# emiliofidalgo/liodom

Measured on AMD Instinct MI355X. Metric: scans/sec (64×1800 cloud, prev_frames=20) at 1 GPU; pose RMSE vs CPU ref, higher is better.
Workload: dtype f64

## Files before the change

### liodom_amd/csrc/kernels_lm.h

```cpp
constexpr int kLmWaves = kLmThreads / 64;


__device__ int lm_compact_bits(const DevView& v, int s, int outer_it, int E, int* idx ) {
  const int lane = threadIdx.x & 63;
  const int Q = v.knn_queries;
  const int nb = (E + Q - 1) / Q;
  const int nwords = (nb + 3) >> 2;
  const unsigned int* mw = reinterpret_cast<const unsigned int*>(v.corr_mask + ((size_t)s * 2 + outer_it) * v.mask_stride);
  int run = 0;
  for (int w0 = 0; w0 < nwords; w0 += 64) {
    const int w = w0 + lane;
    unsigned int word = (w < nwords) ? mw[w] : 0u;
    const int pop = __popc(word);
    const int incl = wave_incl_scan_i32(pop);
    int o = run + incl - pop;
    while (word) {
      const int b = __ffs(word) - 1;
      word &= word - 1u;
      const int bit = w * 32 + b;
      idx[o++] = (bit >> 3) * Q + (bit & 7);
    }
    run += readlane_i32(incl, 63);
  }
  return run;
// ... 325 lines not shown
  __shared__ int sh_spec_at;
  if (threadIdx.x == 77) sh_spec_at = st.spec_eval[outer_it];
  __shared__ int sh_redo;
  if (threadIdx.x == 78) sh_redo = st.spec_redo[outer_it == 0 ? 1 : 0];
  extern __shared__ __attribute__((aligned(16))) int sh_idx[];
  const int tid = threadIdx.x;
  const bool prep = tid < kLmCtl;
  bool dead = false;
  if (chain && outer_it == 0) dead = !chain_wait_count(v.knn_done0 + s, done_target, &st.status);
  if (chain && outer_it == 0 && sh_redo) __builtin_amdgcn_fence(__ATOMIC_ACQUIRE, "agent");
  int E_in;
  if (chain && outer_it == 0) {
    typedef __attribute__((address_space(1))) unsigned int gu32;
    E_in = (int)__hip_atomic_load((gu32*)(v.edge_cnt + eb * 32 + s), __ATOMIC_RELAXED, __HIP_MEMORY_SCOPE_AGENT);
  } else {
    E_in = st.n_edges_buf[eb];
  }
  if (outer_it == 0 && tid == 0 && g == 0) {
    st.info.n_edges = E_in;
    st.info.map_points = st.n_search;
    for (int k = 0; k < 2; k++) {
      st.info.lm[k].iterations = 0; st.info.lm[k].accepted = 0; st.info.lm[k].termination = LM_TERM_NO_RESIDUALS;
      st.info.lm[k].pad = 0; st.info.lm[k].initial_cost = 0.0; st.info.lm[k].final_cost = 0.0;
    }
  }
  if (!st.initialized) {
    if (outer_it == 1 && g == 0) {
      if (seq) ov_wait_knn_done(v, s, seq, &st.status);
      if (tid == 0) st.append_raw = 1;
      __shared__ double sh_T0[12];
      if (tid < 12) sh_T0[tid] = st.odom[tid];
      __syncthreads();
      finalize_scan(v, s, st, sh_cnt, eb, true, 0, 0, sh_T0, 1, true, sh_prev, sh_fc);
      if (tid == 0) st.initialized = 1;
      if (v.cov_raw && tid == 64) {
        PoseCovRaw* r = v.cov_raw + s;
        r->scan_index = st.info.scan_index; r->n_res = 0; r->termination = st.info.lm[1].termination; r->has_solve = 0; r->cost = st.info.lm[1].final_cost;
      }
    }
    return;
  }
  bool clr_pending = outer_it == 1 && g == 0 && prep && !v.early_rebuild;
  auto clear_hash_slots = [&]() {
    hash_clear_used(v, s, st.n_used_tab[0], tid, kLmCtl);
    clr_pending = false;
  };
  const bool dbgb = (s == 0) && (g == 0) && (tid == kLmCtl) && (outer_it == 1);
  const bool dbge = (s == 0) && (g == 0) && (tid == 0) && (outer_it == 1);
  DBG_STAMP(v, dbgb, 2, 0);
  const int E = E_in;
  int nblocks = st.info.matches[outer_it];
  __shared__ int sh_nmatch;
  __shared__ double sh_scale[8];
  const unsigned int epoch0 = ((unsigned int)(st.scan_counter + 1) << 6) | ((unsigned int)outer_it << 5);
  unsigned int n_eval = 0;
  bool xch_local = false;
  LmCache cache;
  int c_lo = 0, c_hi = 0;
  int dbg_it = 0;
  auto evaluate = [&](const double* pose) {
    lm_eval(v, s, outer_it, eb, c_lo, c_hi, sh_idx, pose, &sh_wsum[0][0], cache);
    if (tid >= kLmCtl) {
      const int lane = tid - kLmCtl;
      if (G > 1) {
        const double x = lm_wave_total(&sh_wsum[0][0], c_hi - c_lo, lane >> 1);
        DBG_STAMP(v, dbgb && dbg_it < 4, 2, 12 + dbg_it);
        xch_local = lm_exchange(v, s, g, G, epoch0 | ++n_eval, x, sh_acc, &st.status, xch_local, lane);
      } else {
        if (lane < kAccN) sh_acc[lane] = lm_wave_total(&sh_wsum[0][0], c_hi - c_lo, lane);
        ++n_eval;
      }
      asm volatile("s_waitcnt lgkmcnt(0)" ::: "memory");
      __builtin_amdgcn_wave_barrier();
    }
  };
  auto my_share = [&](int C) {
    const int chunk = (C + G - 1) / G;
    c_lo = g * chunk < C ? g * chunk : C;
    c_hi = (g + 1) * chunk < C ? (g + 1) * chunk : C;
  };
  if (seq && outer_it == 1) { if (chain) dead = !chain_wait_count(v.knn_done0 + 32 + s, done_target, &st.status) || dead; else ov_wait_knn_done(v, s, seq, &st.status); }
  if (seq && outer_it == 1) { __syncthreads(); if (sh_redo) __builtin_amdgcn_fence(__ATOMIC_ACQUIRE, "agent"); }
  OV_STAMP(v, g == 0 && tid == 0 && outer_it == 1, 4);
  OV_STAMP(v, g == 0 && tid == 0 && outer_it == 0, 18);
  if (v.knn_partials) {
    const int Q = v.knn_queries;
    const int nb = (E + Q - 1) / Q;
    const double* part = v.knn_part + ((size_t)s * 2 + outer_it) * v.knn_blocks * 32;
    constexpr int kRC = kLmThreads / 32;
    const int i = tid & 31, r0 = tid >> 5;
    double x0 = 0.0, x1 = 0.0;
    if (i <= kAccN) {
      const int nb_cap = v.knn_blocks;
      for (int rb = r0; rb < (dead ? 0 : (rb == r0 ? nb_cap : nb)); rb += 16 * kRC) {
        double xs[16];
#pragma unroll
        for (int u = 0; u < 16; u++) { const int r = rb + kRC * u; xs[u] = (r < nb_cap) ? part[(size_t)r * 32 + i] : 0.0; }
#pragma unroll
        for (int u = 0; u < 16; u++) { const int r = rb + kRC * u; if (r >= nb) xs[u] = 0.0; }
#pragma unroll
        for (int u = 0; u < 16; u += 2) { x0 += xs[u]; x1 += xs[u + 1]; }
      }
    }
    sh_red[r0][i] = x0 + x1;
    __syncthreads();
    if (tid <= kAccN) {
      double x = 0.0;
#pragma unroll
      for (int r = 0; r < kRC; r++) x += sh_red[r][tid];
      if (tid < kAccN) sh_acc[tid] = x;
      else { sh_nmatch = (int)x; if (g == 0) st.info.matches[outer_it] = (int)x; }
    }
    __syncthreads();
    nblocks = sh_nmatch;
  } else {
    __syncthreads();
    if (prep) {
      const int C = lm_compact_bits(v, s, outer_it, E, sh_idx);
      if (tid == 0) sh_C = C;
    } else if (tid == kLmCtl) {
      iso_from_qt(sh_x0, sh_x0 + 4, sh_pose2[0]);
    }
    __syncthreads();
    my_share(sh_C);
    lm_cache_load(v, s, outer_it, eb, c_lo, c_hi, sh_idx, cache);
    evaluate(sh_pose2[0]);
  }
  DBG_STAMP(v, dbgb, 2, 2);
  int pi = 0, ci = -1, nmoved = 0;
  const unsigned int n_eval0 = n_eval;
  const bool spec_ok = v.speculate != 0 && v.speculate != 5 && v.speculate != 7 && g == 0 && seq != 0u && outer_it == 0;
  const bool spec_ok1 = v.speculate != 0 && v.speculate != 4 && v.speculate != 6 && g == 0 && chain != 0 && outer_it == 1 && v.early_rebuild && v.pred_xch != nullptr;
  const bool spec_forced = v.speculate == 2 || v.speculate == 6 || v.speculate == 7;
  bool spec_done = false;
  int spec_moves = -1;
  for (int step = 0;; step++) {
    if (step == 0 && tid > kLmCtl && tid <= kLmCtl + 6) {
      const int j = tid - kLmCtl - 1;
      sh_scale[j] = 1.0 / (1.0 + sqrt(sh_acc[7 + h_idx(j, j)]));
    }
    if (step == 0) __builtin_amdgcn_wave_barrier();
    if (tid == kLmCtl) {
      const int acc_before = step == 0 ? 0 : lm.accepted;
      const int f = step == 0 ? lm_begin(lm, sh_x0, sh_x0 + 4, sh_acc, nblocks, v.apply_on_ftol, sh_scale) : lm_update(lm, sh_acc);
      sh_flag = f;
      bool moved = step > 0 && lm.accepted != acc_before;
      if (step > 0 && !moved && f != LM_NEED_EVAL && lm.termination == LM_TERM_FUNC_TOL) {
        moved = true;
        for (int k = 0; k < 4; k++) moved = moved && lm.q[k] == lm.cand_q[k];
        for (int k = 0; k < 3; k++) moved = moved && lm.t[k] == lm.cand_t[k];
      }
      if (moved) { ci = pi; pi ^= 1; nmoved++; }
      if (f == LM_NEED_EVAL) iso_from_qt(lm.cand_q, lm.cand_t, sh_pose2[pi]);
      sh_pi = pi; sh_ci = ci; sh_nmoved = nmoved; sh_unapplied = (step > 0 && !moved) ? 1 : 0;
      if (step == 0) DBG_STAMP(v, dbgb, 2, 23);
    } else if (!prep) {
    } else if (step == 0 && v.knn_partials) {
      DBG_STAMP(v, dbge, 2, 24);
      const int C = dead ? 0 : lm_compact_bits(v, s, outer_it, E, sh_idx);
      if (tid == 0) sh_C = C;
      DBG_STAMP(v, dbge, 2, 25);
      my_share(C);
      lm_cache_load(v, s, outer_it, eb, c_lo, c_hi, sh_idx, cache);
    } else if (clr_pending) {
      clear_hash_slots();
    }
    __syncthreads();
    if (step == 0) { if (v.knn_partials && !prep) my_share(sh_C); DBG_STAMP(v, dbgb, 2, 3); }
    else { DBG_STAMP(v, dbgb && dbg_it < 5, 2, 5 + 2 * dbg_it); dbg_it++; }
    if (sh_flag != LM_NEED_EVAL) break;
    if ((spec_ok || spec_ok1) && !spec_done && sh_ci >= 0 &&
        (spec_forced || (!spec_forced && sh_spec_at == 0 && lm.model_cost_change <= v.spec_theta * 1e-6 * lm.cost))) {
      if (spec_ok) {
        ov_publish_pose(v, s, sh_pose2[sh_ci], &lm.q[0], seq, tid, 1);
        OV_STAMP(v, tid == 0, 19);
      } else if (tid >= kLmCtl) {
        const int l = tid - kLmCtl;
        if (l < 25) publish_final_pose(v, s, sh_pose2[sh_ci], 0, (unsigned int)sh_fc + 1u, l, 0);
        if (l == 0) predict_next(sh_pose2[sh_ci], sh_prev, v.rotation_mode, sh_pred_s);
        asm volatile("s_waitcnt lgkmcnt(0)" ::: "memory");
        __builtin_amdgcn_wave_barrier();
        pred_publish(v, s, sh_pred_s, (unsigned int)sh_fc + 1u, l, 64, 1);
        OV_STAMP(v, l == 0, 22);
      }
      if ((kInstrument && (v.debug & 64)) && tid == 0) atomicAdd(&v.dbg_clk[270], 1ull);
      spec_done = true;
      spec_moves = sh_nmoved;
    }
    const double* pose_c = sh_pose2[sh_pi];
    evaluate(pose_c);
    DBG_STAMP(v, dbgb && dbg_it < 5, 2, 4 + 2 * dbg_it);
  }
  if (clr_pending) clear_hash_slots();
  DBG_STAMP(v, dbgb, 2, 20);
  if ((kInstrument && (v.debug & 32)) && dbgb) v.dbg_clk[2 * 32 + 27] = (xch_local ? 100ull : 0ull) + 10ull * xcc_id() + (unsigned long long)n_eval;
  if (g != 0) return;
  __shared__ double sh_ov[20];
  __shared__ liodom_lm_trace_t sh_trace;
  {
    if (tid == kLmCtl) {
      sh_trace.iterations = lm.iter; sh_trace.accepted = lm.accepted; sh_trace.termination = lm.termination; sh_trace.pad = 0;
      sh_trace.initial_cost = lm.initial_cost; sh_trace.final_cost = lm.cost;
    }
    const int cif = sh_ci;
    if (cif >= 0) {
      if (tid < 12) sh_ov[tid] = sh_pose2[cif][tid];
      else if (tid >= 64 && tid < 71) sh_ov[12 + tid - 64] = (&lm.q[0])[tid - 64];
    } else if (tid == kLmCtl) {
      double q[4], t[3], T[12];
      for (int k = 0; k < 4; k++) q[k] = lm.q[k];
      for (int k = 0; k < 3; k++) t[k] = lm.t[k];
      iso_from_qt(q, t, T);
      for (int k = 0; k < 12; k++) sh_ov[k] = T[k];
      for (int k = 0; k < 4; k++) sh_ov[12 + k] = q[k];
      for (int k = 0; k < 3; k++) sh_ov[16 + k] = t[k];
    }
  }
  __syncthreads();
  if (outer_it == 0) {
    if (seq) { ov_publish_pose(v, s, sh_ov, sh_ov + 12, seq, tid, spec_done ? 2 : 3); OV_STAMP(v, tid == 0, 1); }
// ... 25 lines not shown
```

### liodom_amd/csrc/liodom_math.h

```cpp
#pragma once
#include <cfloat>
#include <cmath>
#include <cstdint>

#if defined(__HIPCC__)
#define LD_HD __host__ __device__ __forceinline__
#define LD_UNROLL _Pragma("unroll")
#define LD_FP_CONTRACT_FAST _Pragma("clang fp contract(fast)")
#else
#define LD_HD inline
#define LD_UNROLL
#define LD_FP_CONTRACT_FAST
#endif
#if defined(__HIP_DEVICE_COMPILE__)
#define LD_RSQRT(x) rsqrt(x)
#else
#define LD_RSQRT(x) (1.0 / sqrt(x))
#endif

namespace liodom_dev {

constexpr int kJacobiSweeps = 8;
constexpr int kLmMaxIterations = 4;
constexpr double kHuberA = 0.2;
// ... 238 lines not shown
  m[6] = -sj;     m[7] = cj * si;      m[8] = cj * ci;
}
LD_HD void tf_quat_from_matrix(const double* m, double* q) {
  const double trace = m[0] + m[4] + m[8];
  if (trace > 0.0) {
    double s = sqrt(trace + 1.0);
    q[3] = s * 0.5;
    s = 0.5 / s;
    q[0] = (m[7] - m[5]) * s;
    q[1] = (m[2] - m[6]) * s;
    q[2] = (m[3] - m[1]) * s;
  } else {
    const int i = m[0] < m[4] ? (m[4] < m[8] ? 2 : 1) : (m[0] < m[8] ? 2 : 0);
    const int j = (i + 1) % 3, k = (i + 2) % 3;
    double s = sqrt(m[i * 3 + i] - m[j * 3 + j] - m[k * 3 + k] + 1.0);
    q[i] = s * 0.5;
    s = 0.5 / s;
    q[3] = (m[k * 3 + j] - m[j * 3 + k]) * s;
    q[j] = (m[j * 3 + i] + m[i * 3 + j]) * s;
    q[k] = (m[k * 3 + i] + m[i * 3 + k]) * s;
  }
}
LD_HD void imu_override(const double* odom, const double* imu_q, const double* laser_to_base, int rotation_mode, double* out) {
  double m[9], imu_roll, imu_pitch, imu_yaw, bl_roll, bl_pitch, bl_yaw;
  tf_matrix_from_quat(imu_q, m);
  tf_get_rpy(m, &imu_roll, &imu_pitch, &imu_yaw);
  double odom_bl[12], q_bl[4], q_new[4], l2b_inv[12];
  iso_mul(odom, laser_to_base, odom_bl);
  quat_from_pose(odom_bl, rotation_mode, q_bl);
  tf_matrix_from_quat(q_bl, m);
  tf_get_rpy(m, &bl_roll, &bl_pitch, &bl_yaw);
  tf_set_rpy(imu_roll, imu_pitch, bl_yaw, m);
  tf_quat_from_matrix(m, q_new);
  const double t_bl[3] = {odom_bl[3], odom_bl[7], odom_bl[11]};
  iso_from_qt(q_new, t_bl, odom_bl);
  iso_inverse(laser_to_base, l2b_inv);
  iso_mul(odom_bl, l2b_inv, out);
}
LD_HD void odom_message(const double* prev_odom, const double* odom, const double* laser_to_base,
                        double delta_time, int rotation_mode, double* out) {
  double bl[12], pbl[12], pinv[12], d[12], qd[4], m[9], roll, pitch, yaw;
  iso_mul(odom, laser_to_base, bl);
  quat_from_pose(bl, rotation_mode, out);
  out[4] = bl[3]; out[5] = bl[7]; out[6] = bl[11];
  iso_mul(prev_odom, laser_to_base, pbl);
  iso_inverse(pbl, pinv);
  iso_mul(pinv, bl, d);
  out[7] = d[3] / delta_time; out[8] = d[7] / delta_time; out[9] = d[11] / delta_time;
  quat_from_pose(d, rotation_mode, qd);
  tf_matrix_from_quat(qd, m);
  tf_get_rpy(m, &roll, &pitch, &yaw);
  out[10] = roll / delta_time; out[11] = pitch / delta_time; out[12] = yaw / delta_time;
}
LD_HD void quat_plus(const double* x, const double* delta, double* out) {
  LD_FP_CONTRACT_FAST
  const double u2 = delta[0] * delta[0] + delta[1] * delta[1] + delta[2] * delta[2];
  if (u2 > 0.0) {
    double s, aw;
    if (u2 < 0.25) {
      const double u = u2;
      s = 1.0 + u * (-1.0 / 6.0 + u * (1.0 / 120.0 + u * (-1.0 / 5040.0 + u * (1.0 / 362880.0 + u * (-1.0 / 39916800.0 +
          u * (1.0 / 6227020800.0 + u * (-1.0 / 1307674368000.0 + u * (1.0 / 355687428096000.0))))))));
      aw = 1.0 + u * (-0.5 + u * (1.0 / 24.0 + u * (-1.0 / 720.0 + u * (1.0 / 40320.0 + u * (-1.0 / 3628800.0 +
           u * (1.0 / 479001600.0 + u * (-1.0 / 87178291200.0 + u * (1.0 / 20922789888000.0))))))));
    } else {
      const double nd = sqrt(u2);
      s = sin(nd) / nd;
      aw = cos(nd);
    }
    const double ax = s * delta[0], ay = s * delta[1], az = s * delta[2];
    const double bw = x[3], bx = x[0], by = x[1], bz = x[2];
    out[3] = aw * bw - ax * bx - ay * by - az * bz;
    out[0] = aw * bx + ax * bw + ay * bz - az * by;
    out[1] = aw * by + ay * bw + az * bx - ax * bz;
    out[2] = aw * bz + az * bw + ax * by - ay * bx;
  } else {
    out[0] = x[0]; out[1] = x[1]; out[2] = x[2]; out[3] = x[3];
  }
}

LD_HD float sqdist_f(float qx, float qy, float qz, float mx, float my, float mz) {
  const float dx = qx - mx, dy = qy - my, dz = qz - mz;
  float r = dx * dx;
  r = r + dy * dy;
  r = r + dz * dz;
  return r;
}

LD_HD void jacobi_rot(double& app, double& aqq, double& apq, double& arp, double& arq) {
  if (fabs(apq) <= 1e-20 * (fabs(app) + fabs(aqq))) return;
  const double theta = (aqq - app) / (2.0 * apq);
  const double at = fabs(theta);
  double t = 1.0 / (at + sqrt(theta * theta + 1.0));
  if (theta < 0.0) t = -t;
  const double c = 1.0 / sqrt(t * t + 1.0);
  const double s = t * c;
  app = app - t * apq;
  aqq = aqq + t * apq;
  apq = 0.0;
  const double nrp = c * arp - s * arq;
  const double nrq = s * arp + c * arq;
  arp = nrp; arq = nrq;
}
LD_HD void eig3_sym(const double* a, double* ev) {
  double a00 = a[0], a01 = a[1], a02 = a[2], a11 = a[3], a12 = a[4], a22 = a[5];
  for (int sweep = 0; sweep < kJacobiSweeps; sweep++) {
    jacobi_rot(a00, a11, a01, a02, a12);
    jacobi_rot(a00, a22, a02, a01, a12);
    jacobi_rot(a11, a22, a12, a01, a02);
  }
  double e0 = a00, e1 = a11, e2 = a22, s;
  if (e0 > e1) { s = e0; e0 = e1; e1 = s; }
  if (e1 > e2) { s = e1; e1 = e2; e2 = s; }
  if (e0 > e1) { s = e0; e0 = e1; e1 = s; }
  ev[0] = e0; ev[1] = e1; ev[2] = e2;
}
LD_HD bool line_gate(const float* nx, const float* ny, const float* nz) {
  double cx = 0, cy = 0, cz = 0;
  for (int j = 0; j < 5; j++) { cx = cx + (double)nx[j]; cy = cy + (double)ny[j]; cz = cz + (double)nz[j]; }
  cx = cx / 5.0; cy = cy / 5.0; cz = cz / 5.0;
  double cov[6] = {0, 0, 0, 0, 0, 0};
  for (int j = 0; j < 5; j++) {
    const double zx = (double)nx[j] - cx, zy = (double)ny[j] - cy, zz = (double)nz[j] - cz;
    cov[0] = cov[0] + zx * zx; cov[1] = cov[1] + zx * zy; cov[2] = cov[2] + zx * zz;
    cov[3] = cov[3] + zy * zy; cov[4] = cov[4] + zy * zz; cov[5] = cov[5] + zz * zz;
  }
  const double p1 = cov[1] * cov[1] + cov[2] * cov[2] + cov[4] * cov[4];
  const double q = (cov[0] + cov[3] + cov[5]) / 3.0;
// ... 127 lines not shown
  double scale[6];
  double diag[6];
  double radius, decrease_factor;
  double x_norm;
  double model_cost_change;
  double initial_cost;
  int reuse_diagonal;
  int iter, accepted, invalid_run, termination;
  int apply_on_ftol;
};


LD_HD int lt_idx(int i, int j) { return i * (i + 1) / 2 + j; }
LD_HD bool chol_solve6_packed(double* A , const double* b, double* y) {
  LD_FP_CONTRACT_FAST
  double inv[6];
  LD_UNROLL
  for (int j = 0; j < 6; j++) {
    double d = A[lt_idx(j, j)];
    LD_UNROLL
    for (int k = 0; k < j; k++) d -= A[lt_idx(j, k)] * A[lt_idx(j, k)];
    if (!(d > 0.0) || !ld_isfinite(d)) return false;
#if defined(__HIP_DEVICE_COMPILE__)
    inv[j] = rsqrt(d);
#else
    inv[j] = 1.0 / sqrt(d);
#endif
    LD_UNROLL
    for (int i = j + 1; i < 6; i++) {
      double s = A[lt_idx(i, j)];
      LD_UNROLL
      for (int k = 0; k < j; k++) s -= A[lt_idx(i, k)] * A[lt_idx(j, k)];
      A[lt_idx(i, j)] = s * inv[j];
    }
  }
  double z[6];
  LD_UNROLL
  for (int i = 0; i < 6; i++) {
    double s = b[i];
    LD_UNROLL
    for (int k = 0; k < i; k++) s -= A[lt_idx(i, k)] * z[k];
    z[i] = s * inv[i];
  }
  LD_UNROLL
  for (int i = 5; i >= 0; i--) {
    double s = z[i];
    LD_UNROLL
    for (int k = i + 1; k < 6; k++) s -= A[lt_idx(k, i)] * y[k];
    y[i] = s * inv[i];
    if (!ld_isfinite(y[i])) return false;
  }
  return true;
}

constexpr unsigned int kCovValid = 1u, kCovSingular = 2u, kCovNoSolve = 4u, kCovEvalFailure = 8u, kCovFewResiduals = 16u;
constexpr int kCovJacobiSweeps = 12;

LD_HD bool spd_inverse6(const double* H21, double* inv36) {
  double L[21];
  LD_UNROLL
  for (int i = 0; i < 6; i++) {
    LD_UNROLL
    for (int j = 0; j <= i; j++) L[lt_idx(i, j)] = H21[h_idx(j, i)];
  }
  bool ok = true;
  LD_UNROLL
  for (int j = 0; j < 6; j++) {
    double d = L[lt_idx(j, j)];
    LD_UNROLL
    for (int k = 0; k < j; k++) d -= L[lt_idx(j, k)] * L[lt_idx(j, k)];
    ok = ok && d > 0.0 && ld_isfinite(d);
    const double ljj = sqrt(d);
    L[lt_idx(j, j)] = ljj;
    LD_UNROLL
    for (int i = j + 1; i < 6; i++) {
      double s = L[lt_idx(i, j)];
      LD_UNROLL
      for (int k = 0; k < j; k++) s -= L[lt_idx(i, k)] * L[lt_idx(j, k)];
      L[lt_idx(i, j)] = s / ljj;
    }
  }
  if (!ok) return false;
  double Li[21];
  LD_UNROLL
  for (int j = 0; j < 6; j++) {
    Li[lt_idx(j, j)] = 1.0 / L[lt_idx(j, j)];
    LD_UNROLL
    for (int i = j + 1; i < 6; i++) {
      double s = 0.0;
      LD_UNROLL
      for (int k = j; k < i; k++) s -= L[lt_idx(i, k)] * Li[lt_idx(k, j)];
      Li[lt_idx(i, j)] = s / L[lt_idx(i, i)];
    }
  }
  LD_UNROLL
  for (int i = 0; i < 6; i++) {
    LD_UNROLL
    for (int j = i; j < 6; j++) {
      double s = 0.0;
      LD_UNROLL
      for (int k = j; k < 6; k++) s += Li[lt_idx(k, i)] * Li[lt_idx(k, j)];
      inv36[i * 6 + j] = s;
      inv36[j * 6 + i] = s;
    }
  }
  return true;
// ... 91 lines not shown
    LD_UNROLL
    for (int j = 0; j < 6; j++) info36[i * 6 + j] = h_at(H21, i, j);
  }
  sym_eig6(info36, evals6, evecs36);
  double inv[36];
  if (!spd_inverse6(H21, inv)) return flags | kCovSingular;
  if ((flags & kCovValid) && !(flags & kCovFewResiduals)) {
    LD_UNROLL
    for (int i = 0; i < 36; i++) cov36[i] = *sigma2 * inv[i];
  }
  return flags;
}

LD_HD void pose_cov_to_ros(const double* cov36_tangent, const double* T12, const double* L12, double* out36) {
  double u[3];
  LD_UNROLL
  for (int i = 0; i < 3; i++) u[i] = T12[4 * i] * L12[3] + T12[4 * i + 1] * L12[7] + T12[4 * i + 2] * L12[11];
  double A[36];
  LD_UNROLL
  for (int i = 0; i < 36; i++) A[i] = 0.0;
  A[0 * 6 + 1] = 2.0 * u[2];  A[0 * 6 + 2] = -2.0 * u[1];
  A[1 * 6 + 0] = -2.0 * u[2]; A[1 * 6 + 2] = 2.0 * u[0];
  A[2 * 6 + 0] = 2.0 * u[1];  A[2 * 6 + 1] = -2.0 * u[0];
  LD_UNROLL
  for (int i = 0; i < 3; i++) { A[i * 6 + 3 + i] = 1.0; A[(3 + i) * 6 + i] = 2.0; }
  double AS[36];
  LD_UNROLL
  for (int i = 0; i < 6; i++) {
    LD_UNROLL
    for (int j = 0; j < 6; j++) {
      double s = 0.0;
      LD_UNROLL
      for (int k = 0; k < 6; k++) s += A[i * 6 + k] * cov36_tangent[k * 6 + j];
      AS[i * 6 + j] = s;
    }
  }
  LD_UNROLL
  for (int i = 0; i < 6; i++) {
    LD_UNROLL
    for (int j = 0; j < 6; j++) {
      double s = 0.0;
      LD_UNROLL
      for (int k = 0; k < 6; k++) s += AS[i * 6 + k] * A[j * 6 + k];
      out36[i * 6 + j] = s;
    }
  }
}

LD_HD double norm7(const double* q, const double* t) {
  LD_FP_CONTRACT_FAST
  return sqrt(q[0] * q[0] + q[1] * q[1] + q[2] * q[2] + q[3] * q[3] + t[0] * t[0] + t[1] * t[1] + t[2] * t[2]);
}

LD_HD int lm_propose(LmState& st) {
  LD_FP_CONTRACT_FAST
  while (true) {
    if (st.iter >= kLmMaxIterations) { st.termination = LM_TERM_MAX_ITER; return LM_DONE; }
    if (st.radius < 1e-32) { st.termination = LM_TERM_RADIUS; return LM_DONE; }
    st.iter++;
    double sc[6], gs[6];
    LD_UNROLL
    for (int i = 0; i < 6; i++) { sc[i] = st.scale[i]; gs[i] = sc[i] * st.g[i]; }
    double A[21];
    LD_UNROLL
    for (int i = 0; i < 6; i++) {
      LD_UNROLL
      for (int j = 0; j <= i; j++) A[lt_idx(i, j)] = sc[i] * sc[j] * st.H[h_idx(j, i)];
    }
    if (!st.reuse_diagonal) {
      LD_UNROLL
      for (int j = 0; j < 6; j++) {
        double d = A[lt_idx(j, j)];
        if (d < 1e-6) d = 1e-6;
        if (d > 1e32) d = 1e32;
        st.diag[j] = d;
      }
    }
    const double inv_radius = 1.0 / st.radius;
    LD_UNROLL
    for (int j = 0; j < 6; j++) A[lt_idx(j, j)] += st.diag[j] * inv_radius;
    double y[6];
    const bool ok = chol_solve6_packed(A, gs, y);
    st.reuse_diagonal = 1;
    double mcc = 0.0;
    double step[6];
    if (ok) {
      double sg = 0.0, shs = 0.0;
      LD_UNROLL
      for (int i = 0; i < 6; i++) step[i] = -y[i];
      LD_UNROLL
      for (int i = 0; i < 6; i++) {
        sg += step[i] * gs[i];
        double row = 0.0;
        LD_UNROLL
        for (int j = 0; j < i; j++) row += (sc[i] * sc[j] * st.H[h_idx(j, i)]) * step[j];
        shs += step[i] * (2.0 * row + (sc[i] * sc[i] * st.H[h_idx(i, i)]) * step[i]);
      }
      mcc = -sg - 0.5 * shs;
    }
    if (!ok || !(mcc > 0.0)) {
      if (++st.invalid_run >= 5) { st.termination = LM_TERM_INVALID_STEPS; return LM_DONE; }
      st.radius = st.radius * 0.5;
      continue;
    }
    st.invalid_run = 0;
    st.model_cost_change = mcc;
    double delta[6];
    LD_UNROLL
    for (int j = 0; j < 6; j++) delta[j] = step[j] * sc[j];
    quat_plus(st.q, delta, st.cand_q);
    LD_UNROLL
    for (int k = 0; k < 3; k++) st.cand_t[k] = st.t[k] + delta[3 + k];
    return LM_NEED_EVAL;
  }
}

LD_HD int lm_begin(LmState& st, const double* q0, const double* t0, const double* acc,
                   int n_blocks, int apply_on_ftol, const double* pre_scale = nullptr) {
  LD_UNROLL
  for (int k = 0; k < 4; k++) st.q[k] = st.cand_q[k] = q0[k];
  LD_UNROLL
  for (int k = 0; k < 3; k++) st.t[k] = st.cand_t[k] = t0[k];
  st.iter = 0; st.accepted = 0; st.invalid_run = 0; st.termination = LM_TERM_MAX_ITER;
  st.apply_on_ftol = apply_on_ftol;
  st.cost = 0.0; st.initial_cost = 0.0; st.model_cost_change = 0.0;
  st.radius = 1e4; st.decrease_factor = 2.0; st.reuse_diagonal = 0;
  LD_UNROLL
  for (int j = 0; j < 6; j++) { st.scale[j] = 1.0; st.diag[j] = 0.0; st.g[j] = 0.0; }
  LD_UNROLL
  for (int j = 0; j < 21; j++) st.H[j] = 0.0;
  st.x_norm = norm7(st.q, st.t);
  if (n_blocks == 0) { st.termination = LM_TERM_NO_RESIDUALS; return LM_DONE; }
  if (acc[28] != 0.0) { st.termination = LM_TERM_EVAL_FAILURE; return LM_DONE; }
  st.cost = acc[0]; st.initial_cost = acc[0];
  double gmax = 0.0;
  LD_UNROLL
  for (int j = 0; j < 6; j++) { st.g[j] = acc[1 + j]; const double ag = fabs(st.g[j]); if (ag > gmax) gmax = ag; }
  LD_UNROLL
  for (int j = 0; j < 21; j++) st.H[j] = acc[7 + j];
  LD_UNROLL
  for (int j = 0; j < 6; j++) st.scale[j] = pre_scale ? pre_scale[j] : 1.0 / (1.0 + sqrt(st.H[h_idx(j, j)]));
  if (gmax <= 1e-10) { st.termination = LM_TERM_GRAD_TOL; return LM_DONE; }
  return lm_propose(st);
}

LD_HD int lm_update(LmState& st, const double* acc) {
  LD_FP_CONTRACT_FAST
  const double cand_cost = (acc[28] != 0.0) ? DBL_MAX : acc[0];
  double dq[4], dt[3];
  LD_UNROLL
  for (int k = 0; k < 4; k++) dq[k] = st.q[k] - st.cand_q[k];
  LD_UNROLL
  for (int k = 0; k < 3; k++) dt[k] = st.t[k] - st.cand_t[k];
  const double step_sq = dq[0] * dq[0] + dq[1] * dq[1] + dq[2] * dq[2] + dq[3] * dq[3] + dt[0] * dt[0] + dt[1] * dt[1] + dt[2] * dt[2];
  const double ptol = 1e-8 * (st.x_norm + 1e-8);
  const double ptol_sq = ptol * ptol;
  bool ptol_hit = step_sq <= ptol_sq * (1.0 - 1e-12);
  if (!ptol_hit && step_sq <= ptol_sq * (1.0 + 1e-12)) ptol_hit = sqrt(step_sq) <= ptol;
  if (ptol_hit) { st.termination = LM_TERM_PARAM_TOL; return LM_DONE; }
  const double cost_change = st.cost - cand_cost;
  if (fabs(cost_change) <= 1e-6 * st.cost) {
    st.termination = LM_TERM_FUNC_TOL;
    if (st.apply_on_ftol && cost_change > 0.0) {
      LD_UNROLL
      for (int k = 0; k < 4; k++) st.q[k] = st.cand_q[k];
      LD_UNROLL
      for (int k = 0; k < 3; k++) st.t[k] = st.cand_t[k];
      st.cost = cand_cost;
    }
    return LM_DONE;
  }
  const double rel = cost_change / st.model_cost_change;
  if (rel > 1e-3) {
    LD_UNROLL
    for (int k = 0; k < 4; k++) st.q[k] = st.cand_q[k];
    LD_UNROLL
    for (int k = 0; k < 3; k++) st.t[k] = st.cand_t[k];
    st.x_norm = norm7(st.q, st.t);
    st.cost = cand_cost;
    double gmax = 0.0;
    LD_UNROLL
    for (int j = 0; j < 6; j++) { st.g[j] = acc[1 + j]; const double ag = fabs(st.g[j]); if (ag > gmax) gmax = ag; }
    LD_UNROLL
    for (int j = 0; j < 21; j++) st.H[j] = acc[7 + j];
    st.accepted++;
    const double c = 2.0 * rel - 1.0;
    double f = 1.0 - c * c * c;
    if (f < 1.0 / 3.0) f = 1.0 / 3.0;
    st.radius = st.radius / f;
    if (st.radius > 1e16) st.radius = 1e16;
    st.decrease_factor = 2.0;
    st.reuse_diagonal = 0;
    if (gmax <= 1e-10) { st.termination = LM_TERM_GRAD_TOL; return LM_DONE; }
  } else {
    st.radius = st.radius / st.decrease_factor;
    st.decrease_factor *= 2.0;
    st.reuse_diagonal = 1;
  }
  return lm_propose(st);
}

LD_HD void pg_quat_mul(const double* a, const double* b, double* o) {
  o[3] = a[3] * b[3] - a[0] * b[0] - a[1] * b[1] - a[2] * b[2];
  o[0] = a[3] * b[0] + a[0] * b[3] + a[1] * b[2] - a[2] * b[1];
  o[1] = a[3] * b[1] + a[1] * b[3] + a[2] * b[0] - a[0] * b[2];
  o[2] = a[3] * b[2] + a[2] * b[3] + a[0] * b[1] - a[1] * b[0];
}
LD_HD void pg_rot3(const double* q, double* R ) {
  const double x = q[0], y = q[1], z = q[2], w = q[3];
  const double tx = 2 * x, ty = 2 * y, tz = 2 * z;
  const double twx = tx * w, twy = ty * w, twz = tz * w;
  const double txx = tx * x, txy = ty * x, txz = tz * x;
  const double tyy = ty * y, tyz = tz * y, tzz = tz * z;
  R[0] = 1 - (tyy + tzz); R[1] = txy - twz;       R[2] = txz + twy;
  R[3] = txy + twz;       R[4] = 1 - (txx + tzz); R[5] = tyz - twx;
  R[6] = txz - twy;       R[7] = tyz + twx;       R[8] = 1 - (txx + tyy);
}
LD_HD void graph_edge_error(const double* Xi, const double* Xj, const double* Z, double* e, double* A, double* B) {
  double Ri[9], Rz[9];
  pg_rot3(Xi, Ri);
  pg_rot3(Z, Rz);
  const double u[3] = {Xj[4] - Xi[4], Xj[5] - Xi[5], Xj[6] - Xi[6]};
  double m[3];
  LD_UNROLL
  for (int r = 0; r < 3; r++) m[r] = (Ri[r] * u[0] + Ri[3 + r] * u[1] + Ri[6 + r] * u[2]) - Z[4 + r];
  const double ci[4] = {-Xi[0], -Xi[1], -Xi[2], Xi[3]}, cz[4] = {-Z[0], -Z[1], -Z[2], Z[3]};
  double a[4], qd[4];
  pg_quat_mul(cz, ci, a);
  pg_quat_mul(a, Xj, qd);
  const double s = qd[3] >= 0.0 ? 1.0 : -1.0;
  LD_UNROLL
  for (int r = 0; r < 3; r++) {
    e[r] = s * qd[r];
    e[3 + r] = Rz[r] * m[0] + Rz[3 + r] * m[1] + Rz[6 + r] * m[2];
  }
  if (!A || !B) return;
  double W[9];
  LD_UNROLL
  for (int r = 0; r < 3; r++) {
    LD_UNROLL
    for (int c = 0; c < 3; c++) W[r * 3 + c] = Rz[r] * Ri[c * 3] + Rz[3 + r] * Ri[c * 3 + 1] + Rz[6 + r] * Ri[c * 3 + 2];
  }
  LD_UNROLL
  for (int i = 0; i < 36; i++) { A[i] = 0.0; B[i] = 0.0; }
  LD_UNROLL
  for (int k = 0; k < 3; k++) {
    const double ek[4] = {k == 0 ? 1.0 : 0.0, k == 1 ? 1.0 : 0.0, k == 2 ? 1.0 : 0.0, 0.0};
    double c[4], d[4];
    pg_quat_mul(a, ek, c);
    pg_quat_mul(c, Xj, d);
    LD_UNROLL
    for (int r = 0; r < 3; r++) { B[r * 6 + k] = s * d[r]; A[r * 6 + k] = -(s * d[r]); }
// ... 124 lines not shown
```

Baseline: 14940.

## Add straight-line register fast path for LM begin/update proposal step

Adds a branch-light fast path for the single-thread LM controller. It loads the accumulators and state into registers, precomputes the scale products across 21 threads into shared memory, and runs an unpivoted Cholesky solve with rsqrt. The small-angle quaternion update is applied speculatively. When any termination, rejection or large-rotation condition could apply, it falls back to the original general path. The aim is to shorten the serial controller's critical path between evaluations, in exchange for code size, register pressure and extra timing instrumentation hooks.

```diff
diff --git a/liodom_amd/csrc/kernels_lm.h b/liodom_amd/csrc/kernels_lm.h
--- a/liodom_amd/csrc/kernels_lm.h
+++ b/liodom_amd/csrc/kernels_lm.h
@@ -401,6 +401,7 @@
   int nblocks = st.info.matches[outer_it];
   __shared__ int sh_nmatch;
   __shared__ double sh_scale[8];
+  __shared__ double sh_ss[24];
   const unsigned int epoch0 = ((unsigned int)(st.scan_counter + 1) << 6) | ((unsigned int)outer_it << 5);
   unsigned int n_eval = 0;
   bool xch_local = false;
@@ -483,15 +484,32 @@
   const bool spec_forced = v.speculate == 2 || v.speculate == 6 || v.speculate == 7;
   bool spec_done = false;
   int spec_moves = -1;
+  const bool ctl_budget = kInstrument && (v.debug & 1024) && s == 0 && g == 0;
+  const int ctl_general = (kInstrument && (v.debug & 2048)) ? 1 : 0;
+  unsigned long long t_bar = 0ull;
   for (int step = 0;; step++) {
-    if (step == 0 && tid > kLmCtl && tid <= kLmCtl + 6) {
-      const int j = tid - kLmCtl - 1;
-      sh_scale[j] = 1.0 / (1.0 + sqrt(sh_acc[7 + h_idx(j, j)]));
+    if (ctl_budget) t_bar = wall_clock64();
+    if (step == 0 && tid > kLmCtl && tid <= kLmCtl + 21) {
+      const int k = tid - kLmCtl - 1;
+      int i = 0;
+      while ((i + 1) * (i + 2) / 2 <= k) i++;
+      const int j = k - i * (i + 1) / 2;
+      const double si = 1.0 / (1.0 + sqrt(sh_acc[7 + h_idx(i, i)])), sj = 1.0 / (1.0 + sqrt(sh_acc[7 + h_idx(j, j)]));
+      sh_ss[k] = si * sj;
+      if (i == j) sh_scale[i] = si;
     }
     if (step == 0) __builtin_amdgcn_wave_barrier();
     if (tid == kLmCtl) {
       const int acc_before = step == 0 ? 0 : lm.accepted;
-      const int f = step == 0 ? lm_begin(lm, sh_x0, sh_x0 + 4, sh_acc, nblocks, v.apply_on_ftol, sh_scale) : lm_update(lm, sh_acc);
+      double cand[7];
+      unsigned long long marks_a[LM_MARK_N + 2];
+#pragma unroll
+      for (int k = 0; k < LM_MARK_N + 2; k++) marks_a[k] = 0ull;
+      auto ctl_step = [&](unsigned long long* marks) {
+        return step == 0 ? lm_begin(lm, sh_x0, sh_x0 + 4, sh_acc, nblocks, v.apply_on_ftol, sh_scale, sh_ss, cand, marks, ctl_general)
+                         : lm_update(lm, sh_acc, sh_ss, cand, marks, ctl_general);
+      };
+      const int f = ctl_budget ? ctl_step(marks_a) : ctl_step(nullptr);
       sh_flag = f;
       bool moved = step > 0 && lm.accepted != acc_before;
       if (step > 0 && !moved && f != LM_NEED_EVAL && lm.termination == LM_TERM_FUNC_TOL) {
@@ -500,21 +518,35 @@
         for (int k = 0; k < 3; k++) moved = moved && lm.t[k] == lm.cand_t[k];
       }
       if (moved) { ci = pi; pi ^= 1; nmoved++; }
-      if (f == LM_NEED_EVAL) iso_from_qt(lm.cand_q, lm.cand_t, sh_pose2[pi]);
+      if (f == LM_NEED_EVAL) iso_from_qt(cand, cand + 4, sh_pose2[pi]);
       sh_pi = pi; sh_ci = ci; sh_nmoved = nmoved; sh_unapplied = (step > 0 && !moved) ? 1 : 0;
       if (step == 0) DBG_STAMP(v, dbgb, 2, 23);
+      if (ctl_budget) {
+        marks_a[LM_MARK_N] = wall_clock64();
+        unsigned long long* b = v.dbg_clk + 192 + ((outer_it * 4 + (step < 3 ? step : 3)) * 12);
+#pragma unroll
+        for (int k = 0; k <= LM_MARK_N; k++) if (marks_a[k]) b[k] += marks_a[k] - t_bar;
+        b[11] += 1ull;
+      }
     } else if (!prep) {
     } else if (step == 0 && v.knn_partials) {
       DBG_STAMP(v, dbge, 2, 24);
       const int C = dead ? 0 : lm_compact_bits(v, s, outer_it, E, sh_idx);
       if (tid == 0) sh_C = C;
       DBG_STAMP(v, dbge, 2, 25);
+      const unsigned long long t_cmp = (ctl_budget && tid == 0) ? wall_clock64() : 0ull;
       my_share(C);
       lm_cache_load(v, s, outer_it, eb, c_lo, c_hi, sh_idx, cache);
+      if (ctl_budget && tid == 0) {
+        asm volatile("s_waitcnt vmcnt(0)" ::: "memory");
+        unsigned long long* b = v.dbg_clk + 288 + outer_it * 4;
+        b[0] += t_cmp - t_bar; b[1] += wall_clock64() - t_bar; b[2] += 1ull;
+      }
     } else if (clr_pending) {
       clear_hash_slots();
     }
     __syncthreads();
+    if (ctl_budget && tid == kLmCtl) v.dbg_clk[192 + ((outer_it * 4 + (step < 3 ? step : 3)) * 12) + LM_MARK_N + 1] += wall_clock64() - t_bar;
     if (step == 0) { if (v.knn_partials && !prep) my_share(sh_C); DBG_STAMP(v, dbgb, 2, 3); }
     else { DBG_STAMP(v, dbgb && dbg_it < 5, 2, 5 + 2 * dbg_it); dbg_it++; }
     if (sh_flag != LM_NEED_EVAL) break;
diff --git a/liodom_amd/csrc/liodom_math.h b/liodom_amd/csrc/liodom_math.h
--- a/liodom_amd/csrc/liodom_math.h
+++ b/liodom_amd/csrc/liodom_math.h
@@ -314,28 +314,35 @@
   tf_get_rpy(m, &roll, &pitch, &yaw);
   out[10] = roll / delta_time; out[11] = pitch / delta_time; out[12] = yaw / delta_time;
 }
+LD_HD void quat_small_sincos(double u, double& s, double& aw) {
+  LD_FP_CONTRACT_FAST
+  s = 1.0 + u * (-1.0 / 6.0 + u * (1.0 / 120.0 + u * (-1.0 / 5040.0 + u * (1.0 / 362880.0 + u * (-1.0 / 39916800.0 +
+      u * (1.0 / 6227020800.0 + u * (-1.0 / 1307674368000.0 + u * (1.0 / 355687428096000.0))))))));
+  aw = 1.0 + u * (-0.5 + u * (1.0 / 24.0 + u * (-1.0 / 720.0 + u * (1.0 / 40320.0 + u * (-1.0 / 3628800.0 +
+       u * (1.0 / 479001600.0 + u * (-1.0 / 87178291200.0 + u * (1.0 / 20922789888000.0))))))));
+}
+LD_HD void quat_plus_apply(const double* x, const double* delta, double s, double aw, double* out) {
+  LD_FP_CONTRACT_FAST
+  const double ax = s * delta[0], ay = s * delta[1], az = s * delta[2];
+  const double bw = x[3], bx = x[0], by = x[1], bz = x[2];
+  out[3] = aw * bw - ax * bx - ay * by - az * bz;
+  out[0] = aw * bx + ax * bw + ay * bz - az * by;
+  out[1] = aw * by + ay * bw + az * bx - ax * bz;
+  out[2] = aw * bz + az * bw + ax * by - ay * bx;
+}
 LD_HD void quat_plus(const double* x, const double* delta, double* out) {
   LD_FP_CONTRACT_FAST
   const double u2 = delta[0] * delta[0] + delta[1] * delta[1] + delta[2] * delta[2];
   if (u2 > 0.0) {
     double s, aw;
     if (u2 < 0.25) {
-      const double u = u2;
-      s = 1.0 + u * (-1.0 / 6.0 + u * (1.0 / 120.0 + u * (-1.0 / 5040.0 + u * (1.0 / 362880.0 + u * (-1.0 / 39916800.0 +
-          u * (1.0 / 6227020800.0 + u * (-1.0 / 1307674368000.0 + u * (1.0 / 355687428096000.0))))))));
-      aw = 1.0 + u * (-0.5 + u * (1.0 / 24.0 + u * (-1.0 / 720.0 + u * (1.0 / 40320.0 + u * (-1.0 / 3628800.0 +
-           u * (1.0 / 479001600.0 + u * (-1.0 / 87178291200.0 + u * (1.0 / 20922789888000.0))))))));
+      quat_small_sincos(u2, s, aw);
     } else {
       const double nd = sqrt(u2);
       s = sin(nd) / nd;
       aw = cos(nd);
     }
-    const double ax = s * delta[0], ay = s * delta[1], az = s * delta[2];
-    const double bw = x[3], bx = x[0], by = x[1], bz = x[2];
-    out[3] = aw * bw - ax * bx - ay * by - az * bz;
-    out[0] = aw * bx + ax * bw + ay * bz - az * by;
-    out[1] = aw * by + ay * bw + az * bx - ax * bz;
-    out[2] = aw * bz + az * bw + ax * by - ay * bx;
+    quat_plus_apply(x, delta, s, aw, out);
   } else {
     out[0] = x[0]; out[1] = x[1]; out[2] = x[2]; out[3] = x[3];
   }
@@ -569,6 +576,43 @@
   }
   return true;
 }
+LD_HD bool chol_solve6_packed_straight(double* A , const double* b, double* y) {
+  LD_FP_CONTRACT_FAST
+  double inv[6];
+  bool ok = true;
+  LD_UNROLL
+  for (int j = 0; j < 6; j++) {
+    double d = A[lt_idx(j, j)];
+    LD_UNROLL
+    for (int k = 0; k < j; k++) d -= A[lt_idx(j, k)] * A[lt_idx(j, k)];
+    ok = ok & (d > 0.0) & ld_isfinite(d);
+    inv[j] = LD_RSQRT(d);
+    LD_UNROLL
+    for (int i = j + 1; i < 6; i++) {
+      double s = A[lt_idx(i, j)];
+      LD_UNROLL
+      for (int k = 0; k < j; k++) s -= A[lt_idx(i, k)] * A[lt_idx(j, k)];
+      A[lt_idx(i, j)] = s * inv[j];
+    }
+  }
+  double z[6];
+  LD_UNROLL
+  for (int i = 0; i < 6; i++) {
+    double s = b[i];
+    LD_UNROLL
+    for (int k = 0; k < i; k++) s -= A[lt_idx(i, k)] * z[k];
+    z[i] = s * inv[i];
+  }
+  LD_UNROLL
+  for (int i = 5; i >= 0; i--) {
+    double s = z[i];
+    LD_UNROLL
+    for (int k = i + 1; k < 6; k++) s -= A[lt_idx(k, i)] * y[k];
+    y[i] = s * inv[i];
+    ok = ok & ld_isfinite(y[i]);
+  }
+  return ok;
+}
 
 constexpr unsigned int kCovValid = 1u, kCovSingular = 2u, kCovNoSolve = 4u, kCovEvalFailure = 8u, kCovFewResiduals = 16u;
 constexpr int kCovJacobiSweeps = 12;
@@ -766,7 +810,15 @@
   return sqrt(q[0] * q[0] + q[1] * q[1] + q[2] * q[2] + q[3] * q[3] + t[0] * t[0] + t[1] * t[1] + t[2] * t[2]);
 }
 
-LD_HD int lm_propose(LmState& st) {
+enum { LM_MARK_LOADED = 0, LM_MARK_DECIDED = 1, LM_MARK_SCALED = 2, LM_MARK_SOLVED = 3, LM_MARK_MCC = 4, LM_MARK_CAND = 5,
+       LM_MARK_STORED = 6, LM_MARK_GENERAL = 7, LM_MARK_N = 8 };
+#if defined(__HIP_DEVICE_COMPILE__)
+#define LD_LM_MARK(m, k) do { if (m) (m)[k] = wall_clock64(); } while (0)
+#else
+#define LD_LM_MARK(m, k) do { if (m) (m)[k] = 1ull; } while (0)
+#endif
+
+LD_HD int lm_propose_general(LmState& st, unsigned long long* marks = nullptr) {
   LD_FP_CONTRACT_FAST
   while (true) {
     if (st.iter >= kLmMaxIterations) { st.termination = LM_TERM_MAX_ITER; return LM_DONE; }
@@ -793,8 +845,10 @@
     const double inv_radius = 1.0 / st.radius;
     LD_UNROLL
     for (int j = 0; j < 6; j++) A[lt_idx(j, j)] += st.diag[j] * inv_radius;
+    LD_LM_MARK(marks, LM_MARK_SCALED);
     double y[6];
     const bool ok = chol_solve6_packed(A, gs, y);
+    LD_LM_MARK(marks, LM_MARK_SOLVED);
     st.reuse_diagonal = 1;
     double mcc = 0.0;
     double step[6];
@@ -812,6 +866,7 @@
       }
       mcc = -sg - 0.5 * shs;
     }
+    LD_LM_MARK(marks, LM_MARK_MCC);
     if (!ok || !(mcc > 0.0)) {
       if (++st.invalid_run >= 5) { st.termination = LM_TERM_INVALID_STEPS; return LM_DONE; }
       st.radius = st.radius * 0.5;
@@ -825,12 +880,14 @@
     quat_plus(st.q, delta, st.cand_q);
     LD_UNROLL
     for (int k = 0; k < 3; k++) st.cand_t[k] = st.t[k] + delta[3 + k];
+    LD_LM_MARK(marks, LM_MARK_CAND);
     return LM_NEED_EVAL;
   }
 }
 
-LD_HD int lm_begin(LmState& st, const double* q0, const double* t0, const double* acc,
-                   int n_blocks, int apply_on_ftol, const double* pre_scale = nullptr) {
+LD_HD int lm_begin_general(LmState& st, const double* q0, const double* t0, const double* acc,
+                           int n_blocks, int apply_on_ftol, const double* pre_scale = nullptr, unsigned long long* marks = nullptr) {
+  LD_LM_MARK(marks, LM_MARK_GENERAL);
   LD_UNROLL
   for (int k = 0; k < 4; k++) st.q[k] = st.cand_q[k] = q0[k];
   LD_UNROLL
@@ -854,12 +911,14 @@
   for (int j = 0; j < 21; j++) st.H[j] = acc[7 + j];
   LD_UNROLL
   for (int j = 0; j < 6; j++) st.scale[j] = pre_scale ? pre_scale[j] : 1.0 / (1.0 + sqrt(st.H[h_idx(j, j)]));
+  LD_LM_MARK(marks, LM_MARK_DECIDED);
   if (gmax <= 1e-10) { st.termination = LM_TERM_GRAD_TOL; return LM_DONE; }
-  return lm_propose(st);
-}
-
-LD_HD int lm_update(LmState& st, const double* acc) {
+  return lm_propose_general(st, marks);
+}
+
+LD_HD int lm_update_general(LmState& st, const double* acc, unsigned long long* marks = nullptr) {
   LD_FP_CONTRACT_FAST
+  LD_LM_MARK(marks, LM_MARK_GENERAL);
   const double cand_cost = (acc[28] != 0.0) ? DBL_MAX : acc[0];
   double dq[4], dt[3];
   LD_UNROLL
@@ -911,7 +970,221 @@
     st.decrease_factor *= 2.0;
     st.reuse_diagonal = 1;
   }
-  return lm_propose(st);
+  LD_LM_MARK(marks, LM_MARK_DECIDED);
+  return lm_propose_general(st, marks);
+}
+
+
+struct LmRegs {
+  double q[4], t[3];
+  double g[6], H[21];
+  double sc[6], ss[21];
+  double radius;
+  double diag[6], mcc, cand_q[4], cand_t[3];
+};
+
+LD_HD void lm_scale_products(const double* sc, double* ss ) {
+  LD_UNROLL
+  for (int i = 0; i < 6; i++) {
+    LD_UNROLL
+    for (int j = 0; j <= i; j++) ss[lt_idx(i, j)] = sc[i] * sc[j];
+  }
+}
+
+LD_HD bool lm_propose_regs(LmRegs& r, unsigned long long* marks) {
+  LD_FP_CONTRACT_FAST
+  double gs[6];
+  LD_UNROLL
+  for (int i = 0; i < 6; i++) gs[i] = r.sc[i] * r.g[i];
+  double As[21], A[21];
+  LD_UNROLL
+  for (int i = 0; i < 6; i++) {
+    LD_UNROLL
+    for (int j = 0; j <= i; j++) As[lt_idx(i, j)] = r.ss[lt_idx(i, j)] * r.H[h_idx(j, i)];
+  }
+  LD_UNROLL
+  for (int j = 0; j < 6; j++) {
+    double d = As[lt_idx(j, j)];
+    d = d < 1e-6 ? 1e-6 : d;
+    d = d > 1e32 ? 1e32 : d;
+    r.diag[j] = d;
+  }
+  const double inv_radius = 1.0 / r.radius;
+  LD_UNROLL
+  for (int k = 0; k < 21; k++) A[k] = As[k];
+  LD_UNROLL
+  for (int j = 0; j < 6; j++) A[lt_idx(j, j)] += r.diag[j] * inv_radius;
+  LD_LM_MARK(marks, LM_MARK_SCALED);
+  double y[6];
+  bool ok = chol_solve6_packed_straight(A, gs, y);
+  LD_LM_MARK(marks, LM_MARK_SOLVED);
+  double step[6];
+  double sg = 0.0, shs = 0.0;
+  LD_UNROLL
+  for (int i = 0; i < 6; i++) step[i] = -y[i];
+  LD_UNROLL
+  for (int i = 0; i < 6; i++) {
+    sg += step[i] * gs[i];
+    double row = 0.0;
+    LD_UNROLL
+    for (int j = 0; j < i; j++) row += As[lt_idx(i, j)] * step[j];
+    shs += step[i] * (2.0 * row + As[lt_idx(i, i)] * step[i]);
+  }
+  r.mcc = -sg - 0.5 * shs;
+  ok = ok & (r.mcc > 0.0);
+  LD_LM_MARK(marks, LM_MARK_MCC);
+  double delta[6];
+  LD_UNROLL
+  for (int j = 0; j < 6; j++) delta[j] = step[j] * r.sc[j];
+  const double u2 = delta[0] * delta[0] + delta[1] * delta[1] + delta[2] * delta[2];
+  ok = ok & (u2 > 0.0) & (u2 < 0.25);
+  double s, aw;
+  quat_small_sincos(u2, s, aw);
+  quat_plus_apply(r.q, delta, s, aw, r.cand_q);
+  LD_UNROLL
+  for (int k = 0; k < 3; k++) r.cand_t[k] = r.t[k] + delta[3 + k];
+  LD_LM_MARK(marks, LM_MARK_CAND);
+  return ok;
+}
+
+LD_HD void lm_store_proposal(LmState& st, const LmRegs& r, int iter, double* cand) {
+  LD_UNROLL
+  for (int j = 0; j < 6; j++) { st.g[j] = r.g[j]; st.diag[j] = r.diag[j]; }
+  LD_UNROLL
+  for (int j = 0; j < 21; j++) st.H[j] = r.H[j];
+  LD_UNROLL
+  for (int k = 0; k < 4; k++) { st.q[k] = r.q[k]; st.cand_q[k] = r.cand_q[k]; }
+  LD_UNROLL
+  for (int k = 0; k < 3; k++) { st.t[k] = r.t[k]; st.cand_t[k] = r.cand_t[k]; }
+  st.radius = r.radius; st.decrease_factor = 2.0; st.reuse_diagonal = 1;
+  st.iter = iter; st.invalid_run = 0;
+  st.model_cost_change = r.mcc;
+  if (cand) {
+    LD_UNROLL
+    for (int k = 0; k < 4; k++) cand[k] = r.cand_q[k];
+    LD_UNROLL
+    for (int k = 0; k < 3; k++) cand[4 + k] = r.cand_t[k];
+  }
+}
+LD_HD void lm_cand_from_state(const LmState& st, double* cand) {
+  if (!cand) return;
+  LD_UNROLL
+  for (int k = 0; k < 4; k++) cand[k] = st.cand_q[k];
+  LD_UNROLL
+  for (int k = 0; k < 3; k++) cand[4 + k] = st.cand_t[k];
+}
+
+LD_HD int lm_begin(LmState& st, const double* q0, const double* t0, const double* acc, int n_blocks, int apply_on_ftol,
+                   const double* pre_scale = nullptr, const double* pre_ss = nullptr, double* cand = nullptr,
+                   unsigned long long* marks = nullptr, int general = 0) {
+  LD_FP_CONTRACT_FAST
+  double a[29];
+  LD_UNROLL
+  for (int i = 0; i < 29; i++) a[i] = acc[i];
+  LmRegs r;
+  LD_UNROLL
+  for (int k = 0; k < 4; k++) r.q[k] = q0[k];
+  LD_UNROLL
+  for (int k = 0; k < 3; k++) r.t[k] = t0[k];
+  LD_UNROLL
+  for (int j = 0; j < 6; j++) { r.g[j] = a[1 + j]; }
+  LD_UNROLL
+  for (int j = 0; j < 21; j++) r.H[j] = a[7 + j];
+  LD_UNROLL
+  for (int j = 0; j < 6; j++) r.sc[j] = pre_scale ? pre_scale[j] : 1.0 / (1.0 + sqrt(r.H[h_idx(j, j)]));
+  if (pre_ss) {
+    LD_UNROLL
+    for (int k = 0; k < 21; k++) r.ss[k] = pre_ss[k];
+  } else {
+    lm_scale_products(r.sc, r.ss);
+  }
+  LD_LM_MARK(marks, LM_MARK_LOADED);
+  if (!general && n_blocks != 0 && !(a[28] != 0.0)) {
+    const double x_norm = norm7(r.q, r.t);
+    double gmax = 0.0;
+    LD_UNROLL
+    for (int j = 0; j < 6; j++) { const double ag = fabs(r.g[j]); gmax = ag > gmax ? ag : gmax; }
+    r.radius = 1e4;
+    LD_LM_MARK(marks, LM_MARK_DECIDED);
+    const bool ok = lm_propose_regs(r, marks);
+    if (ok & !(gmax <= 1e-10)) {
+      LD_UNROLL
+      for (int j = 0; j < 6; j++) st.scale[j] = r.sc[j];
+      st.accepted = 0; st.termination = LM_TERM_MAX_ITER; st.apply_on_ftol = apply_on_ftol;
+      st.cost = a[0]; st.initial_cost = a[0]; st.x_norm = x_norm;
+      lm_store_proposal(st, r, 1, cand);
+      LD_LM_MARK(marks, LM_MARK_STORED);
+      return LM_NEED_EVAL;
+    }
+  }
+  const int f = lm_begin_general(st, q0, t0, acc, n_blocks, apply_on_ftol, pre_scale, marks);
+  lm_cand_from_state(st, cand);
+  LD_LM_MARK(marks, LM_MARK_STORED);
+  return f;
+}
+
+LD_HD int lm_update(LmState& st, const double* acc, const double* ss = nullptr, double* cand = nullptr,
+                    unsigned long long* marks = nullptr, int general = 0) {
+  LD_FP_CONTRACT_FAST
+  double a[29];
+  LD_UNROLL
+  for (int i = 0; i < 29; i++) a[i] = acc[i];
+  LmRegs r;
+  double q[4], t[3];
+  LD_UNROLL
+  for (int k = 0; k < 4; k++) { q[k] = st.q[k]; r.q[k] = st.cand_q[k]; }
+  LD_UNROLL
+  for (int k = 0; k < 3; k++) { t[k] = st.t[k]; r.t[k] = st.cand_t[k]; }
+  LD_UNROLL
+  for (int j = 0; j < 6; j++) r.sc[j] = st.scale[j];
+  if (ss) {
+    LD_UNROLL
+    for (int k = 0; k < 21; k++) r.ss[k] = ss[k];
+  } else {
+    lm_scale_products(r.sc, r.ss);
+  }
+  const double cost = st.cost, x_norm_old = st.x_norm, mcc_old = st.model_cost_change, radius = st.radius;
+  const int iter = st.iter, accepted = st.accepted;
+  LD_LM_MARK(marks, LM_MARK_LOADED);
+  double dq[4], dt[3];
+  LD_UNROLL
+  for (int k = 0; k < 4; k++) dq[k] = q[k] - r.q[k];
+  LD_UNROLL
+  for (int k = 0; k < 3; k++) dt[k] = t[k] - r.t[k];
+  const double step_sq = dq[0] * dq[0] + dq[1] * dq[1] + dq[2] * dq[2] + dq[3] * dq[3] + dt[0] * dt[0] + dt[1] * dt[1] + dt[2] * dt[2];
+  const double ptol = 1e-8 * (x_norm_old + 1e-8);
+  const double ptol_sq = ptol * ptol;
+  const double cand_cost = a[0];
+  const double cost_change = cost - cand_cost;
+  const bool may_end = (a[28] != 0.0) | (step_sq <= ptol_sq * (1.0 + 1e-12)) | (fabs(cost_change) <= 1e-6 * cost);
+  if (!general && !may_end) {
+    const double rel = cost_change / mcc_old;
+    const double x_norm = norm7(r.q, r.t);
+    double gmax = 0.0;
+    LD_UNROLL
+    for (int j = 0; j < 6; j++) { r.g[j] = a[1 + j]; const double ag = fabs(r.g[j]); gmax = ag > gmax ? ag : gmax; }
+    LD_UNROLL
+    for (int j = 0; j < 21; j++) r.H[j] = a[7 + j];
+    const double c = 2.0 * rel - 1.0;
+    double f = 1.0 - c * c * c;
+    f = f < 1.0 / 3.0 ? 1.0 / 3.0 : f;
+    double rad = radius / f;
+    rad = rad > 1e16 ? 1e16 : rad;
+    r.radius = rad;
+    LD_LM_MARK(marks, LM_MARK_DECIDED);
+    bool ok = (rel > 1e-3) & !(gmax <= 1e-10) & !(iter >= kLmMaxIterations) & !(rad < 1e-32);
+    ok = ok & lm_propose_regs(r, marks);
+    if (ok) {
+      st.x_norm = x_norm; st.cost = cand_cost; st.accepted = accepted + 1;
+      lm_store_proposal(st, r, iter + 1, cand);
+      LD_LM_MARK(marks, LM_MARK_STORED);
+      return LM_NEED_EVAL;
+    }
+  }
+  const int fl = lm_update_general(st, acc, marks);
+  lm_cand_from_state(st, cand);
+  LD_LM_MARK(marks, LM_MARK_STORED);
+  return fl;
 }
 
 LD_HD void pg_quat_mul(const double* a, const double* b, double* o) {
```

After: 15510 (median of 4 runs). 3.8% higher.
